# shadygm/Lichtfeld-Densification-Plugin

Measured on AMD Instinct MI355X. Metric: triangulated points/sec + pairs/sec, MipNeRF360 garden @fast, 1/2/4/8 GPU, higher is better.
Workload: dtype f32 (+f64 Sampson/DLT solve)

## Files before the change

lichtfeld-densification-plugin_amd/csrc/lfd_api.hip:

```cpp
#include <cstddef>
#include <hip/hip_runtime.h>
#include <hip/hip_ext.h>

#include <algorithm>
#include <cmath>
#include <cstdio>
#include <cstdlib>
#include <cstring>
#include <mutex>
#include <string>
#include <vector>

#include "lfd_context.hpp"

extern "C" __global__ void lfd_aggregate_kernel(LfdLaunch L, float* best_cert, uint8_t* best_slot);
extern "C" __global__ void lfd_dense_kernel(LfdLaunch L);
extern "C" __global__ void lfd_dense_exact_kernel(LfdLaunch L);
extern "C" __global__ void lfd_dense_ply_kernel(LfdLaunch L);
extern "C" __global__ void lfd_dense_ply_exact_kernel(LfdLaunch L);
extern "C" __global__ void lfd_dense_segments_kernel(LfdLaunch L);
extern "C" __global__ void lfd_dense_segments_exact_kernel(LfdLaunch L);
extern "C" __global__ void lfd_dense_ply_segments_kernel(LfdLaunch L);
extern "C" __global__ void lfd_dense_ply_segments_exact_kernel(LfdLaunch L);
extern "C" __global__ void lfd_segment_scan_kernel(const LfdTileSeg* table, int n_tiles, int tiles_per_ref, int n_refs, long long* tile_dst, long long* ref_offsets);
// ... 1370 lines not shown
    int64_t lo = key(-1.0f), hi = key(1.0f);
    while (hi - lo > 1) {
        const int64_t mid = lo + (hi - lo) / 2;
        if (ok(unkey(mid))) lo = mid; else hi = mid;
    }
    return unkey(lo);
}

int lfd_host_fundamental(const float* K1, const float* R1, const float* t1, const float* K2, const float* R2,
                         const float* t2, float* F_out) {
    if (!K1 || !R1 || !t1 || !K2 || !R2 || !t2 || !F_out) return LFD_ERR_INVALID;
    lfd_fundamental(K1, R1, t1, K2, R2, t2, F_out);
    return LFD_OK;
}

static void unpack_cam(const float* v, LfdCam& c) {
    std::memcpy(c.K, v, 9 * 4); std::memcpy(c.R, v + 9, 9 * 4); std::memcpy(c.t, v + 18, 3 * 4);
    std::memcpy(c.P, v + 21, 12 * 4); std::memcpy(c.C, v + 33, 3 * 4);
    c.w = (int32_t)v[36]; c.h = (int32_t)v[37]; c.pad[0] = c.pad[1] = 0;
}

int lfd_host_null_vector(const float* A16, double* out4) {
    if (!A16 || !out4) return -LFD_ERR_INVALID;
    return lfd_null_vector(A16, out4);
}

int lfd_host_eval_correspondence(const float* cam1, const float* cam2, float xa_norm, float ya_norm, float xb_norm,
                                 float yb_norm, int32_t w_match, int32_t h_match, const lfd_params* params, float* out8) {
    if (!cam1 || !cam2 || !params || !out8 || w_match <= 1 || h_match <= 1) return LFD_ERR_INVALID;
    LfdCam a, b;
    unpack_cam(cam1, a); unpack_cam(cam2, b);
    LfdRefConst rc; LfdPairConst pc;
    lfd_make_ref_const(a, w_match, h_match, rc);
    lfd_make_pair_const(a, b, 1, w_match, h_match, pc);
    lfd_batch bb; std::memset(&bb, 0, sizeof(bb));
    bb.w_match = w_match; bb.h_match = h_match;
    LfdKernelParams kp;
    lfd_fill_kernel_params(&bb, params, kp);
    LfdCellResult res;
    lfd_eval_correspondence(rc, pc, xa_norm, ya_norm, xb_norm, yb_norm, kp, res);
    out8[0] = res.x; out8[1] = res.y; out8[2] = res.z; out8[3] = 0.0f; out8[4] = 0.0f; out8[5] = 0.0f;
    out8[6] = res.err; out8[7] = (float)res.keep;
    return LFD_OK;
}

}
```

lichtfeld-densification-plugin_amd/csrc/lfd_geometry.hpp:

```cpp
#pragma once

#include <math.h>
#include <stdint.h>

#if defined(__HIPCC__)
#define LFD_HD __host__ __device__ __forceinline__
#else
#define LFD_HD inline
#endif
#if defined(__HIP_DEVICE_COMPILE__)
#define LFD_REREAD_CONSTANTS() asm volatile("" ::: "memory")
#define LFD_OPAQUE4(a, b, c, d) asm volatile("" : "+v"(a), "+v"(b), "+v"(c), "+v"(d) :: "memory")
#else
#define LFD_REREAD_CONSTANTS() do { } while (0)
#define LFD_OPAQUE4(a, b, c, d) do { } while (0)
#endif

struct LfdCam {
    float K[9];
    float R[9];
    float t[3];
    float P[12];
    float C[3];
    int32_t w, h;
    int32_t pad[2];
};

struct LfdRefConst {
    float P[12];
    float C[3];
    float sx, sy;
    float pad;
};

struct LfdPairConst {
    double F[9];
    float P[12];
    float C[3];
    float sx, sy;
    int32_t cam;
};

struct LfdKernelParams {
    double sampson_thresh;
    float certainty_thresh;
    float reproj_thresh;
    float dot_thresh;
    float wm1, hm1;
    int32_t use_sampson;
    int32_t use_parallax;
    int32_t no_filter;
};

struct LfdCellResult {
    float x, y, z;
    float err;
    float xa_px, ya_px;
    int32_t keep;
};

struct LfdAxis {
    float start, end, step;
    int32_t half, n;
};

LFD_HD LfdAxis lfd_make_axis(int n) {
    LfdAxis a;
    a.start = (float)(-1.0 + 1.0 / (double)n);
    a.end = (float)(1.0 - 1.0 / (double)n);
    a.step = (n > 1) ? (a.end - a.start) / (float)(n - 1) : 0.0f;
    a.half = n / 2;
    a.n = n;
    return a;
// ... 36 lines not shown
    for (int i = 0; i < 3; ++i)
        for (int j = 0; j < 3; ++j)
            R[i * 3 + j] = lfd_dot3_chain(R2[i * 3 + 0], R1[j * 3 + 0], R2[i * 3 + 1], R1[j * 3 + 1], R2[i * 3 + 2], R1[j * 3 + 2]);
    for (int i = 0; i < 3; ++i) {
        const float rt = (R[i * 3 + 0] * t1[0] + R[i * 3 + 1] * t1[1]) + R[i * 3 + 2] * t1[2];
        t[i] = t2[i] - rt;
    }
    const float S[9] = {0.0f, -t[2], t[1], t[2], 0.0f, -t[0], -t[1], t[0], 0.0f};
    for (int i = 0; i < 3; ++i)
        for (int j = 0; j < 3; ++j)
            E[i * 3 + j] = lfd_dot3_chain(S[i * 3 + 0], R[0 + j], S[i * 3 + 1], R[3 + j], S[i * 3 + 2], R[6 + j]);
    lfd_inv3_intrinsics(K1, K1i);
    lfd_inv3_intrinsics(K2, K2i);
    for (int i = 0; i < 3; ++i)
        for (int j = 0; j < 3; ++j)
            T[i * 3 + j] = lfd_dot3_chain(K2i[0 + i], E[0 + j], K2i[3 + i], E[3 + j], K2i[6 + i], E[6 + j]);
    for (int i = 0; i < 3; ++i)
        for (int j = 0; j < 3; ++j)
            F[i * 3 + j] = lfd_dot3_chain(T[i * 3 + 0], K1i[0 + j], T[i * 3 + 1], K1i[3 + j], T[i * 3 + 2], K1i[6 + j]);
}

LFD_HD void lfd_interleave_p(const float* P, float* Pi) {
    for (int c = 0; c < 4; ++c) { Pi[2 * c] = P[c]; Pi[2 * c + 1] = P[4 + c]; Pi[8 + c] = P[8 + c]; }
}

LFD_HD void lfd_make_ref_const(const LfdCam& c, int w_match, int h_match, LfdRefConst& o) {
    lfd_interleave_p(c.P, o.P);
    for (int i = 0; i < 3; ++i) o.C[i] = c.C[i];
    o.sx = (float)((double)c.w / (double)w_match);
    o.sy = (float)((double)c.h / (double)h_match);
    o.pad = 0.0f;
}

LFD_HD void lfd_make_pair_const(const LfdCam& a, const LfdCam& b, int cam_index, int w_match, int h_match,
                                LfdPairConst& o, const float* F_given = nullptr) {
    float F[9];
    if (F_given) { for (int i = 0; i < 9; ++i) F[i] = F_given[i]; }
    else lfd_fundamental(a.K, a.R, a.t, b.K, b.R, b.t, F);
    for (int i = 0; i < 9; ++i) o.F[i] = (double)F[i];
    lfd_interleave_p(b.P, o.P);
    for (int i = 0; i < 3; ++i) o.C[i] = b.C[i];
    o.sx = (float)((double)b.w / (double)w_match);
    o.sy = (float)((double)b.h / (double)h_match);
    o.cam = cam_index;
}

#ifndef LFD_PACK_ROWS
#define LFD_PACK_ROWS 0
#endif
#ifndef LFD_PARALLAX_EXACT
#define LFD_PARALLAX_EXACT 4
#endif
#ifndef LFD_NULLVEC_TOL
#define LFD_NULLVEC_TOL 1e-6
#endif
#ifndef LFD_NULLVEC_MAXIT
#define LFD_NULLVEC_MAXIT 8
#endif
#ifndef LFD_NULLVEC_PASSES
#define LFD_NULLVEC_PASSES 4
#endif

LFD_HD double lfd_pow2_inv_scale(double t) {
    int e;
    (void)frexp(t, &e);
    int es = ((t > 0.0) && (t < 1.7976931348623157e308)) ? -e : 0;
#if defined(__HIP_DEVICE_COMPILE__)
    asm volatile("" : "+v"(es));
#endif
    return ldexp(1.0, es);
}

#ifndef LFD_RCP_NEWTON_STEPS
#define LFD_RCP_NEWTON_STEPS 1
#endif
LFD_HD double lfd_sqrt_rare(double x) {
#if defined(__HIP_DEVICE_COMPILE__)
    const double r = __builtin_amdgcn_rsq(x);
    double s = x * r, h = 0.5 * r;
    double d = fma(-h, s, 0.5);
    s = fma(s, d, s); h = fma(h, d, h);
    d = fma(-s, s, x);
    s = fma(d, h, s);
    return (x > 0.0) ? s : 0.0;
#else
    return sqrt(x);
#endif
}

LFD_HD double lfd_recip_refined(double d) {
#if defined(__HIP_DEVICE_COMPILE__)
    double r = __builtin_amdgcn_rcp(d);
    r = fma(fma(-d, r, 1.0), r, r);
#if LFD_RCP_NEWTON_STEPS >= 2
    r = fma(fma(-d, r, 1.0), r, r);
#endif
    return r;
#else
    return 1.0 / d;
#endif
}

template <class RowFn>
LFD_HD int lfd_null_vector_rows(RowFn rows, double* c) {
    double m00, m01, m02, m03, m11, m12, m13, m22, m23, m33;
#define LFD_BUILD_M()                                                                                                   \
    {                                                                                                                   \
        float Af[16];                                                                                                   \
        rows(Af);                                                                                                       \
        {                                      \
            const double a0 = (double)Af[0], a1 = (double)Af[1], a2 = (double)Af[2], a3 = (double)Af[3];                \
            m00 = a0 * a0; m01 = a0 * a1; m02 = a0 * a2; m03 = a0 * a3;                                                 \
            m11 = a1 * a1; m12 = a1 * a2; m13 = a1 * a3; m22 = a2 * a2; m23 = a2 * a3; m33 = a3 * a3;                   \
        }                                                                                                               \
        _Pragma("unroll") for (int r = 1; r < 4; ++r) {                                                                 \
            const double a0 = (double)Af[4 * r + 0], a1 = (double)Af[4 * r + 1], a2 = (double)Af[4 * r + 2],            \
                         a3 = (double)Af[4 * r + 3];                                                                    \
            m00 = fma(a0, a0, m00); m01 = fma(a0, a1, m01); m02 = fma(a0, a2, m02); m03 = fma(a0, a3, m03);             \
            m11 = fma(a1, a1, m11); m12 = fma(a1, a2, m12); m13 = fma(a1, a3, m13);                                     \
            m22 = fma(a2, a2, m22); m23 = fma(a2, a3, m23); m33 = fma(a3, a3, m33);                                     \
        }                                                                                                               \
    }
    double sh = 0.0;
    double x0 = 0.0, x1 = 0.0, x2 = 0.0, x3 = 1.0;
    int it = 0;
    for (int pass = 0;; ++pass) {
        LFD_BUILD_M();
        const double q00 = m00 - sh, q11 = m11 - sh, q22 = m22 - sh, q33 = m33 - sh;
        const double r0 = lfd_recip_refined(q00);
        const double l10 = m01 * r0, l20 = m02 * r0, l30 = m03 * r0;
        const double d1 = fma(-l10, m01, q11);
        const double n12 = fma(-l10, m02, m12), n13 = fma(-l10, m03, m13);
        const double n22 = fma(-l20, m02, q22), n23 = fma(-l20, m03, m23), n33 = fma(-l30, m03, q33);
        const double r1 = lfd_recip_refined(d1);
        const double l21 = n12 * r1, l31 = n13 * r1;
        const double d2 = fma(-l21, n12, n22);
        const double p23 = fma(-l21, n13, n23), p33 = fma(-l31, n13, n33);
        const double r2 = lfd_recip_refined(d2);
        const double l32 = p23 * r2;
        const double d3 = fma(-l32, p23, p33);
        const double s0 = d3 * r0, s1 = d3 * r1, s2 = d3 * r2;
        if (pass == 0) {
            x3 = 1.0;
            x2 = -l32;
            x1 = fma(-l21, x2, -l31);
            x0 = fma(-l10, x1, fma(-l20, x2, -l30));
            it = 1;
        }
        bool settled = false;
        for (int k = 1;; ++k) {
            const double o0 = x0, o1 = x1, o2 = x2, o3 = x3;
            const double y1 = fma(-l10, x0, x1);
            const double y2 = fma(-l21, y1, fma(-l20, x0, x2));
            const double y3 = fma(-l32, y2, fma(-l31, y1, fma(-l30, x0, x3)));
            const double z0 = x0 * s0, z1 = y1 * s1, z2 = y2 * s2;
            x3 = y3;
            x2 = fma(-l32, x3, z2);
            x1 = fma(-l21, x2, fma(-l31, x3, z1));
            x0 = fma(-l10, x1, fma(-l20, x2, fma(-l30, x3, z0)));
            ++it;
            if (k >= 2) {
                const double ref = fabs(x3 * o3) * LFD_NULLVEC_TOL;
                const double e0 = fabs(fma(x0, o3, -(x3 * o0))), e1 = fabs(fma(x1, o3, -(x3 * o1))), e2 = fabs(fma(x2, o3, -(x3 * o2)));
                const bool more = (e0 > ref) || (e1 > ref) || (e2 > ref) || !(ref > 0.0);
                const bool bad = !(e0 == e0) || !(e1 == e1) || !(e2 == e2) || !(ref == ref);
                if (!more || bad) { settled = true; break; }
                if (k >= LFD_NULLVEC_MAXIT) break;
            }
        }
        if (settled || pass >= LFD_NULLVEC_PASSES - 1) break;
        LFD_BUILD_M();
        {
            const double sc = lfd_pow2_inv_scale(fabs(x0) + fabs(x1) + fabs(x2) + fabs(x3));
            x0 *= sc; x1 *= sc; x2 *= sc; x3 *= sc;
            const double t0 = fma(m03, x3, fma(m02, x2, fma(m01, x1, m00 * x0)));
            const double t1 = fma(m13, x3, fma(m12, x2, fma(m11, x1, m01 * x0)));
            const double t2 = fma(m23, x3, fma(m22, x2, fma(m12, x1, m02 * x0)));
            const double t3 = fma(m33, x3, fma(m23, x2, fma(m13, x1, m03 * x0)));
            const double num = fma(x3, t3, fma(x2, t2, fma(x1, t1, x0 * t0)));
            const double den = fma(x3, x3, fma(x2, x2, fma(x1, x1, x0 * x0)));
            const double rden = lfd_recip_refined(den);
            const double rho = num * rden;
            const double e0 = fma(-rho, x0, t0), e1 = fma(-rho, x1, t1), e2 = fma(-rho, x2, t2), e3 = fma(-rho, x3, t3);
            const double rr = fma(e3, e3, fma(e2, e2, fma(e1, e1, e0 * e0)));
            sh = rho - lfd_sqrt_rare(rr * rden);
        }
    }
    c[0] = x0; c[1] = x1; c[2] = x2; c[3] = x3;
    return it;
#undef LFD_BUILD_M
}

struct LfdCopyRows {
    const float* A;
    LFD_HD void operator()(float* Af) const { for (int i = 0; i < 16; ++i) Af[i] = A[i]; }
};
LFD_HD int lfd_null_vector(const float* Af, double* c) {
    LfdCopyRows rows{Af};
    return lfd_null_vector_rows(rows, c);
}

LFD_HD double lfd_div_by_recip(double a, double b, double r) {
    const double q = a * r;
    return fma(fma(-b, q, a), r, q);
}

LFD_HD float lfd_match_px(float n, float size_m1) {
    return ((n + 1.0f) * 0.5f) * size_m1;
}

LFD_HD float lfd_div_by_recip_f32(float a, float b, float r) {
    const float q = a * r;
    return fmaf(fmaf(-b, q, a), r, q);
}

LFD_HD float lfd_proj_row(const float* Pi, int row, float X0, float X1, float X2, float X3) {
    if (row == 2) return fmaf(X3, Pi[11], fmaf(X2, Pi[10], fmaf(X1, Pi[9], X0 * Pi[8])));
    return fmaf(X3, Pi[6 + row], fmaf(X2, Pi[4 + row], fmaf(X1, Pi[2 + row], X0 * Pi[row])));
}

// ... 15 lines not shown
LFD_HD float lfd_sqrt_rn_f32(float x) {
#if defined(__HIP_DEVICE_COMPILE__)
    const float s = __builtin_amdgcn_sqrtf(x);
    const float h = 0.5f * __builtin_amdgcn_rcpf(s);
    const float r = fmaf(-s, s, x);
    const float c = fmaf(r, h, s);
    return (x > 0.0f && x < 3.0e38f) ? c : s;
#else
    return sqrtf(x);
#endif
}
LFD_HD float lfd_rcp_rn_f32(float b) {
#if defined(__HIP_DEVICE_COMPILE__)
    const float y = __builtin_amdgcn_rcpf(b);
    return fmaf(fmaf(-b, y, 1.0f), y, y);
#else
    return 1.0f / b;
#endif
}

LFD_HD float lfd_reproj_sq(const float* P, float X0, float X1, float X2, float X3, float u, float v, float& pz) {
    const float px = lfd_proj_row(P, 0, X0, X1, X2, X3);
    const float py = lfd_proj_row(P, 1, X0, X1, X2, X3);
    pz = lfd_proj_row(P, 2, X0, X1, X2, X3);
    const float z = fmaxf(pz, 1e-12f);
    const float rz = lfd_rcp_f32(z);
    const float du = lfd_div_by_recip_f32(px, z, rz) - u;
    const float dv = lfd_div_by_recip_f32(py, z, rz) - v;
    return du * du + dv * dv;
}

LFD_HD bool lfd_finite(float x) { return fabsf(x) <= 3.402823466e+38f; }

LFD_HD void lfd_eval_correspondence(const LfdRefConst& rc, const LfdPairConst& pc, float xan, float yan,
                                    float xbn, float ybn, const LfdKernelParams& kp, LfdCellResult& o) {
    const float xa = lfd_match_px(xan, kp.wm1), ya = lfd_match_px(yan, kp.hm1);
    const float xb = lfd_match_px(xbn, kp.wm1), yb = lfd_match_px(ybn, kp.hm1);
    const float ua = xa * rc.sx, va = ya * rc.sy;
    const float ub = xb * pc.sx, vb = yb * pc.sy;
    o.xa_px = xa; o.ya_px = ya;
    o.x = o.y = o.z = 0.0f; o.err = 0.0f; o.keep = 0;

    if (kp.use_sampson) {
        const double x1 = (double)ua, y1 = (double)va, x2 = (double)ub, y2 = (double)vb;
        const double* F = pc.F;
        const double fx0 = fma(F[1], y1, fma(F[0], x1, F[2]));
        const double fx1 = fma(F[4], y1, fma(F[3], x1, F[5]));
        const double fx2 = fma(F[7], y1, fma(F[6], x1, F[8]));
        const double ft0 = fma(F[3], y2, fma(F[0], x2, F[6]));
        const double ft1 = fma(F[4], y2, fma(F[1], x2, F[7]));
        const double num = fma(x2, fx0, fma(y2, fx1, fx2));
        const double den = fma(ft1, ft1, fma(ft0, ft0, fma(fx1, fx1, fx0 * fx0))) + 1e-12;
        if (!((num * num) < kp.sampson_thresh * den)) return;
    }

    struct Rows {
        const LfdRefConst& rc; const LfdPairConst& pc; float ua, va, ub, vb;
        LFD_HD void operator()(float* A) const {
            float u1 = ua, v1 = va, u2 = ub, v2 = vb;
            LFD_OPAQUE4(u1, v1, u2, v2);
            typedef float v2f __attribute__((ext_vector_type(2)));
            const v2f uv1 = {u1, v1}, uv2 = {u2, v2};
            for (int c = 0; c < 4; ++c) {
#if LFD_PACK_ROWS & 1
                const v2f p1 = {rc.P[2 * c], rc.P[2 * c + 1]};
                const v2f m1 = uv1 * rc.P[8 + c];
                const v2f r1 = m1 - p1;
                A[0 + c] = r1.x; A[4 + c] = r1.y;
#else
                A[0 + c] = u1 * rc.P[8 + c] - rc.P[2 * c];
                A[4 + c] = v1 * rc.P[8 + c] - rc.P[2 * c + 1];
#endif
#if LFD_PACK_ROWS & 2
                const v2f p2 = {pc.P[2 * c], pc.P[2 * c + 1]};
                const v2f m2 = uv2 * pc.P[8 + c];
                const v2f r2 = m2 - p2;
                A[8 + c] = r2.x; A[12 + c] = r2.y;
#else
                A[8 + c] = u2 * pc.P[8 + c] - pc.P[2 * c];
                A[12 + c] = v2 * pc.P[8 + c] - pc.P[2 * c + 1];
#endif
            }
        }
    };
    double c[4];
#if defined(LFD_ABLATE_SOLVER)
    c[0] = ua; c[1] = va; c[2] = ub; c[3] = vb;
// ... 265 lines not shown
```

lichtfeld-densification-plugin_amd/csrc/lfd_host.hip:

```cpp
#include <algorithm>
#include <atomic>
#include <cmath>
#include <condition_variable>
#include <cstring>
#include <functional>
#include <mutex>
#include <thread>
#include <vector>

#include "lfd_context.hpp"

void lfd_fill_kernel_params(const lfd_batch* b, const lfd_params* p, LfdKernelParams& kp);

namespace {

struct HostRef {
    LfdRefConst rc;
    LfdPairConst pc[LFD_MAX_SLOTS];
};

struct HostLaunch {
    const lfd_batch* b;
    LfdKernelParams kp;
    std::vector<float> axis_x, axis_y;
// ... 92 lines not shown
        if (!b->image[r]) return lfd_fail(ctx, LFD_ERR_INVALID, "null image pointer");
        for (int j = 0; j < b->n_slots[r]; ++j) {
            const size_t s = (size_t)r * b->k + j;
            if (b->nbr_cam[s] < 0 || b->nbr_cam[s] >= n_cams) return lfd_fail(ctx, LFD_ERR_INVALID, "nbr_cam out of range");
            if (!b->cert[s] || !b->warp[s]) return lfd_fail(ctx, LFD_ERR_INVALID, "null cert/warp pointer in a valid slot");
        }
    }
    return LFD_OK;
}

void prepare_host(const lfd_batch* b, const lfd_params* p, HostLaunch& L) {
    L.b = b;
    lfd_fill_kernel_params(b, p, L.kp);
    L.HW = b->H * b->W;
    L.mask_sx = (float)b->w_match / (float)b->W;
    L.mask_sy = (float)b->h_match / (float)b->H;
    L.exact_colour = (p->flags & LFD_FLAG_EXACT_COLOUR) != 0;
    if (b->axis_x) { L.ax = b->axis_x; L.ay = b->axis_y; }
    else {
        L.axis_x.resize((size_t)b->W); L.axis_y.resize((size_t)b->H);
        const LfdAxis ax = lfd_make_axis(b->W), ay = lfd_make_axis(b->H);
        for (int j = 0; j < b->W; ++j) L.axis_x[(size_t)j] = lfd_axis_value(ax, j);
        for (int j = 0; j < b->H; ++j) L.axis_y[(size_t)j] = lfd_axis_value(ay, j);
        L.ax = L.axis_x.data(); L.ay = L.axis_y.data();
    }
}

void make_ref(const lfd_context* ctx, const HostLaunch& L, int r, HostRef& R) {
    const lfd_batch* b = L.b;
    const LfdCam& ca = ctx->host_cams[(size_t)b->ref_cam[r]];
    lfd_make_ref_const(ca, b->w_match, b->h_match, R.rc);
    for (int j = 0; j < b->n_slots[r]; ++j) {
        const size_t s = (size_t)r * b->k + j;
        lfd_make_pair_const(ca, ctx->host_cams[(size_t)b->nbr_cam[s]], b->nbr_cam[s], b->w_match, b->h_match, R.pc[j],
                            b->fundamental ? b->fundamental + s * 9 : nullptr);
    }
}

float host_cell_cert(const HostLaunch& L, int r, int j, int cell, int x, int y) {
    const lfd_batch* b = L.b;
    const size_t s = (size_t)r * b->k + j;
    float c = lfd_cert_floor(b->cert[s][cell], L.kp.certainty_thresh);
    const uint8_t* ma = b->mask_a ? b->mask_a[r] : nullptr;
    if (ma) c = c * (float)ma[(size_t)lfd_nearest_src(y, L.mask_sy, b->h_match) * b->w_match + lfd_nearest_src(x, L.mask_sx, b->w_match)];
    const uint8_t* mb = b->mask_b ? b->mask_b[s] : nullptr;
    if (mb) {
        const float* wv = b->warp[s] + (size_t)cell * b->warp_channels + (b->warp_channels - 2);
        const int ix = lfd_grid_nearest(wv[0], b->W), iy = lfd_grid_nearest(wv[1], b->H);
        float m = 0.0f;
        if (ix >= 0 && iy >= 0)
            m = (float)mb[(size_t)lfd_nearest_src(iy, L.mask_sy, b->h_match) * b->w_match + lfd_nearest_src(ix, L.mask_sx, b->w_match)];
        c = c * m;
    }
    return c;
}

void host_cell_best(const HostLaunch& L, int r, int cell, float& best, int& bj) {
    const int y = cell / L.b->W, x = cell - y * L.b->W;
    best = host_cell_cert(L, r, 0, cell, x, y);
    bj = 0;
    for (int j = 1; j < L.b->n_slots[r]; ++j) {
        const float c = host_cell_cert(L, r, j, cell, x, y);
        if ((c > best) || ((c != c) && !(best != best))) { best = c; bj = j; }
    }
}

struct HostPoint { float x, y, z, r, g, b, err; int cell; int slot; };
// ... 194 lines not shown
```

lichtfeld-densification-plugin_amd/csrc/lfd_kernels.hip:

```cpp
#include <hip/hip_runtime.h>
#include <stdint.h>

#include "lfd_device.hpp"

namespace {

constexpr int kBlock = LFD_DENSE_BLOCK;
constexpr int kCpt = LFD_DENSE_CPT;
constexpr int kTile = kBlock * kCpt;

typedef unsigned long long u64;

constexpr u64 kStEmpty = 0ull, kStAggregate = 1ull, kStPrefix = 2ull;
constexpr u64 kValueMask = (1ull << LFD_VALUE_BITS) - 1ull;
__device__ __forceinline__ u64 pack_state(u64 st, unsigned epoch, u64 v) {
    return (st << 62) | ((u64)epoch << LFD_VALUE_BITS) | (v & kValueMask);
}
__device__ __forceinline__ u64 state_status(u64 s, unsigned epoch) {
    return (((s >> LFD_VALUE_BITS) & LFD_EPOCH_MASK) == epoch) ? (s >> 62) : kStEmpty;
}

__device__ __forceinline__ void state_store(u64* p, u64 v) {
    __hip_atomic_store(p, v, __ATOMIC_RELAXED, __HIP_MEMORY_SCOPE_AGENT);
}
// ... 270 lines not shown
#pragma unroll
            for (int e = 0; e < 4; ++e) { best[e] = c[e]; bj[e] = 0; }
        } else {
#pragma unroll
            for (int e = 0; e < 4; ++e) argmax_step(c[e], j, best[e], bj[e]);
        }
    }
}

__device__ __forceinline__ void cell_coords(const LfdLaunch& L, const BlockShared& S, int cell, int bj, float& xan,
                                            float& yan, float& xbn, float& ybn) {
    const float* wp = S.slot[bj].warp;
    if (L.warp_channels == 4) {
        const float4 v = load_f32x4(wp + (size_t)cell * 4);
        xan = v.x; yan = v.y; xbn = v.z; ybn = v.w;
    } else {
        const float2 v = load_f32x2(wp + (size_t)cell * 2);
        int y, x;
        lfd_divmod(cell, L.W, L.inv_w, y, x);
        xan = lfd_global(L.axis_x)[x]; yan = lfd_global(L.axis_y)[y];
        xbn = v.x; ybn = v.y;
    }
}

}

extern "C" __global__ void lfd_pair_setup_kernel(LfdLaunch L, LfdRefConst* __restrict__ ref_out,
                                                 LfdPairConst* __restrict__ pair_out) {
    const int i = (int)(blockIdx.x * blockDim.x + threadIdx.x);
    const int n_pairs = L.n_refs * L.k;
    if (i < n_pairs) {
        const int r = i / L.k, j = i - r * L.k;
        if (j < L.refs[r].n_slots) {
            lfd_make_pair_const(L.cams[L.refs[r].cam], L.cams[L.slots[i].cam], L.slots[i].cam, L.w_match, L.h_match, pair_out[i],
                                L.fund_override ? L.fund_override + (size_t)i * 9 : nullptr);
        }
    } else if (i < n_pairs + L.n_refs) {
        const int r = i - n_pairs;
        lfd_make_ref_const(L.cams[L.refs[r].cam], L.w_match, L.h_match, ref_out[r]);
    }
}

extern "C" __global__ void __launch_bounds__(256) lfd_aggregate_kernel(LfdLaunch L, float* __restrict__ best_cert,
                                                                       uint8_t* __restrict__ best_slot) {
    __shared__ BlockShared S;
    const int r = (int)blockIdx.y;
    const int tid = (int)threadIdx.x;
    if (tid == 0) S.ref = L.refs[r];
    if (tid < L.k) S.slot[tid] = L.slots[(size_t)r * L.k + tid];
    __syncthreads();
    const int HW = L.H * L.W;
    const bool plain = !S.ref.mask_a && (HW & 3) == 0;
    bool any_mask_b = false;
    for (int j = 0; j < S.ref.n_slots; ++j) any_mask_b |= (S.slot[j].mask_b != nullptr);
    const int ns = S.ref.n_slots;
    for (int base = ((int)blockIdx.x * 256 + tid) * 4; base < HW; base += (int)gridDim.x * 256 * 4) {
        if (plain && !any_mask_b && base + 3 < HW) {
            float4 best = load_f32x4(S.slot[0].cert + base);
            const float th = L.kp.certainty_thresh;
            best.x = lfd_cert_floor(best.x, th); best.y = lfd_cert_floor(best.y, th);
            best.z = lfd_cert_floor(best.z, th); best.w = lfd_cert_floor(best.w, th);
            int b0 = 0, b1 = 0, b2 = 0, b3 = 0;
            for (int j = 1; j < ns; ++j) {
                const float4 c = load_f32x4(S.slot[j].cert + base);
                argmax_step(lfd_cert_floor(c.x, th), j, best.x, b0);
                argmax_step(lfd_cert_floor(c.y, th), j, best.y, b1);
                argmax_step(lfd_cert_floor(c.z, th), j, best.z, b2);
// ... 790 lines not shown
```

lichtfeld-densification-plugin_amd/csrc/build.py:

```python
from __future__ import annotations

import os
import shutil
import subprocess
import sys

HERE = os.path.dirname(os.path.abspath(__file__))
OUT = os.path.join(os.path.dirname(HERE), "liblfd_densify.so")
SOURCES = ["lfd_api.hip", "lfd_kernels.hip", "lfd_select.hip", "lfd_writer.hip", "lfd_host.hip", "lfd_image.hip", "lfd_voxel.hip"]
HEADERS = ["lfd_device.hpp", "lfd_geometry.hpp", "lfd_context.hpp", os.path.join("..", "..", "include", "lfd_densify.h")]
FLAGS = ["--offload-arch=gfx950", "-O3", "-std=c++17", "-ffp-contract=off", "-fPIC", "-shared",
         "-fno-fast-math", "-Wall", "-Wno-unused-function", "-pthread", "-mllvm", "-amdgpu-sched-strategy=max-ilp"]


def needs_build() -> bool:
    if not os.path.exists(OUT):
        return True
    t = os.path.getmtime(OUT)
    return any(os.path.getmtime(os.path.join(HERE, f)) > t for f in SOURCES + HEADERS + ["build.py"])


def build(force: bool = False, verbose: bool = False) -> str:
    if not force and not needs_build():
        return OUT
    hipcc = shutil.which("hipcc") or "/opt/rocm/bin/hipcc"
    cmd = [hipcc] + FLAGS + [os.path.join(HERE, s) for s in SOURCES] + ["-o", OUT]
    if verbose:
        cmd.insert(1, "-Rpass-analysis=kernel-resource-usage")
        print(" ".join(cmd))
    res = subprocess.run(cmd, capture_output=True, text=True)
    if res.returncode != 0:
        sys.stderr.write(res.stdout + res.stderr)
        raise RuntimeError("hipcc failed building liblfd_densify.so")
    if verbose:
        sys.stderr.write(res.stderr)
    return OUT


if __name__ == "__main__":
    print(build(force="--force" in sys.argv, verbose="-v" in sys.argv))
```

Before: 50.81 billion.

## Filter Sampson test in f32 with error bound, fall back to f64 when ambiguous

The Sampson epipolar check now runs first in single precision, using per-pair error-bound constants computed at pair setup. Only when the f32 margin is within a rigorous rounding bound, or the coordinates exceed the assumed range, does it recompute in f64. The aim is to avoid the slow f64 FMA chain on MI355X for most cells while keeping decisions identical. The cost is extra per-pair constants in LfdPairConst, a divergent exact path, and a tuned bound that must be correct. It also adds an ISA-mix profiling script.

```diff
diff --git a/lichtfeld-densification-plugin_amd/csrc/lfd_api.hip b/lichtfeld-densification-plugin_amd/csrc/lfd_api.hip
--- a/lichtfeld-densification-plugin_amd/csrc/lfd_api.hip
+++ b/lichtfeld-densification-plugin_amd/csrc/lfd_api.hip
@@ -1426,11 +1426,11 @@
     unpack_cam(cam1, a); unpack_cam(cam2, b);
     LfdRefConst rc; LfdPairConst pc;
     lfd_make_ref_const(a, w_match, h_match, rc);
-    lfd_make_pair_const(a, b, 1, w_match, h_match, pc);
     lfd_batch bb; std::memset(&bb, 0, sizeof(bb));
     bb.w_match = w_match; bb.h_match = h_match;
     LfdKernelParams kp;
     lfd_fill_kernel_params(&bb, params, kp);
+    lfd_make_pair_const(a, b, 1, w_match, h_match, kp.sampson_thresh, pc);
     LfdCellResult res;
     lfd_eval_correspondence(rc, pc, xa_norm, ya_norm, xb_norm, yb_norm, kp, res);
     out8[0] = res.x; out8[1] = res.y; out8[2] = res.z; out8[3] = 0.0f; out8[4] = 0.0f; out8[5] = 0.0f;
diff --git a/lichtfeld-densification-plugin_amd/csrc/lfd_geometry.hpp b/lichtfeld-densification-plugin_amd/csrc/lfd_geometry.hpp
--- a/lichtfeld-densification-plugin_amd/csrc/lfd_geometry.hpp
+++ b/lichtfeld-densification-plugin_amd/csrc/lfd_geometry.hpp
@@ -34,11 +34,13 @@
 };
 
 struct LfdPairConst {
-    double F[9];
+    float F[9];
     float P[12];
     float C[3];
     float sx, sy;
     int32_t cam;
+    float samp_r, samp_t, samp_a1, samp_a0;
+    float pad;
 };
 
 struct LfdKernelParams {
@@ -141,17 +143,39 @@
     o.pad = 0.0f;
 }
 
-LFD_HD void lfd_make_pair_const(const LfdCam& a, const LfdCam& b, int cam_index, int w_match, int h_match,
+LFD_HD void lfd_sampson_consts(const float* F, float R, double t, LfdPairConst& o) {
+    const double u = 5.9604644775390625e-08, tiny = 3.009265538105056e-36;
+    double f[9];
+    for (int i = 0; i < 9; ++i) f[i] = fabs((double)F[i]);
+    const double r = (double)R;
+    const double ax0 = r * (f[0] + f[1]) + f[2], ax1 = r * (f[3] + f[4]) + f[5], ax2 = r * (f[6] + f[7]) + f[8];
+    const double at0 = r * (f[0] + f[3]) + f[6], at1 = r * (f[1] + f[4]) + f[7];
+    const double anum = r * (ax0 + ax1) + ax2;
+    const double en = 4.03 * u * anum + tiny * (4.0 * r + 4.0);
+    const double eS = 8.1 * u * (ax0 * ax0 + ax1 * ax1 + at0 * at0 + at1 * at1) + tiny * (8.0 + 4.0 * (ax0 + ax1 + at0 + at1));
+    const double k = 1.0 + 1.0 / 1024.0;
+    o.samp_r = R;
+    o.samp_t = (float)t;
+    o.samp_a1 = (float)(2.0 * en * k);
+    o.samp_a0 = (float)((en * en + t * (eS + u * 1e-12) + tiny * (1.0 + t)) * k);
+}
+
+LFD_HD void lfd_make_pair_const(const LfdCam& a, const LfdCam& b, int cam_index, int w_match, int h_match, double sampson_thresh,
                                 LfdPairConst& o, const float* F_given = nullptr) {
     float F[9];
     if (F_given) { for (int i = 0; i < 9; ++i) F[i] = F_given[i]; }
     else lfd_fundamental(a.K, a.R, a.t, b.K, b.R, b.t, F);
-    for (int i = 0; i < 9; ++i) o.F[i] = (double)F[i];
+    for (int i = 0; i < 9; ++i) o.F[i] = F[i];
     lfd_interleave_p(b.P, o.P);
     for (int i = 0; i < 3; ++i) o.C[i] = b.C[i];
     o.sx = (float)((double)b.w / (double)w_match);
     o.sy = (float)((double)b.h / (double)h_match);
     o.cam = cam_index;
+    int m = a.w > a.h ? a.w : a.h;
+    if (b.w > m) m = b.w;
+    if (b.h > m) m = b.h;
+    lfd_sampson_consts(F, m > 0 ? 2.0f * (float)m : 0.0f, sampson_thresh, o);
+    o.pad = 0.0f;
 }
 
 #ifndef LFD_PACK_ROWS
@@ -376,6 +400,37 @@
 
 LFD_HD bool lfd_finite(float x) { return fabsf(x) <= 3.402823466e+38f; }
 
+LFD_HD bool lfd_sampson_keep(const LfdPairConst& pc, double thresh, float ua, float va, float ub, float vb, int* exact_path = nullptr) {
+    const float* Ff = pc.F;
+    const float fx0 = fmaf(Ff[1], va, fmaf(Ff[0], ua, Ff[2]));
+    const float fx1 = fmaf(Ff[4], va, fmaf(Ff[3], ua, Ff[5]));
+    const float fx2 = fmaf(Ff[7], va, fmaf(Ff[6], ua, Ff[8]));
+    const float ft0 = fmaf(Ff[3], vb, fmaf(Ff[0], ub, Ff[6]));
+    const float ft1 = fmaf(Ff[4], vb, fmaf(Ff[1], ub, Ff[7]));
+    const float num = fmaf(ub, fx0, fmaf(vb, fx1, fx2));
+    const float den = fmaf(ft1, ft1, fmaf(ft0, ft0, fmaf(fx1, fx1, fx0 * fx0))) + 1e-12f;
+    const float p = pc.samp_t * den;
+    const float d = fmaf(num, num, -p);
+    const float bound = fmaf(pc.samp_a1, fabsf(num), fmaf(4.76837158203125e-07f, p, pc.samp_a0));
+    const float mx = fmaxf(fmaxf(fabsf(ua), fabsf(va)), fmaxf(fabsf(ub), fabsf(vb)));
+    bool pass = d < 0.0f;
+    if (!((mx <= pc.samp_r) && (fabsf(d) > bound))) {
+        if (exact_path) *exact_path = 1;
+        const double x1 = (double)ua, y1 = (double)va, x2 = (double)ub, y2 = (double)vb;
+        double F[9];
+        for (int i = 0; i < 9; ++i) F[i] = (double)Ff[i];
+        const double dfx0 = fma(F[1], y1, fma(F[0], x1, F[2]));
+        const double dfx1 = fma(F[4], y1, fma(F[3], x1, F[5]));
+        const double dfx2 = fma(F[7], y1, fma(F[6], x1, F[8]));
+        const double dft0 = fma(F[3], y2, fma(F[0], x2, F[6]));
+        const double dft1 = fma(F[4], y2, fma(F[1], x2, F[7]));
+        const double dnum = fma(x2, dfx0, fma(y2, dfx1, dfx2));
+        const double dden = fma(dft1, dft1, fma(dft0, dft0, fma(dfx1, dfx1, dfx0 * dfx0))) + 1e-12;
+        pass = (dnum * dnum) < thresh * dden;
+    }
+    return pass;
+}
+
 LFD_HD void lfd_eval_correspondence(const LfdRefConst& rc, const LfdPairConst& pc, float xan, float yan,
                                     float xbn, float ybn, const LfdKernelParams& kp, LfdCellResult& o) {
     const float xa = lfd_match_px(xan, kp.wm1), ya = lfd_match_px(yan, kp.hm1);
@@ -385,18 +440,7 @@
     o.xa_px = xa; o.ya_px = ya;
     o.x = o.y = o.z = 0.0f; o.err = 0.0f; o.keep = 0;
 
-    if (kp.use_sampson) {
-        const double x1 = (double)ua, y1 = (double)va, x2 = (double)ub, y2 = (double)vb;
-        const double* F = pc.F;
-        const double fx0 = fma(F[1], y1, fma(F[0], x1, F[2]));
-        const double fx1 = fma(F[4], y1, fma(F[3], x1, F[5]));
-        const double fx2 = fma(F[7], y1, fma(F[6], x1, F[8]));
-        const double ft0 = fma(F[3], y2, fma(F[0], x2, F[6]));
-        const double ft1 = fma(F[4], y2, fma(F[1], x2, F[7]));
-        const double num = fma(x2, fx0, fma(y2, fx1, fx2));
-        const double den = fma(ft1, ft1, fma(ft0, ft0, fma(fx1, fx1, fx0 * fx0))) + 1e-12;
-        if (!((num * num) < kp.sampson_thresh * den)) return;
-    }
+    if (kp.use_sampson && !lfd_sampson_keep(pc, kp.sampson_thresh, ua, va, ub, vb)) return;
 
     struct Rows {
         const LfdRefConst& rc; const LfdPairConst& pc; float ua, va, ub, vb;
diff --git a/lichtfeld-densification-plugin_amd/csrc/lfd_host.hip b/lichtfeld-densification-plugin_amd/csrc/lfd_host.hip
--- a/lichtfeld-densification-plugin_amd/csrc/lfd_host.hip
+++ b/lichtfeld-densification-plugin_amd/csrc/lfd_host.hip
@@ -148,7 +148,7 @@
     lfd_make_ref_const(ca, b->w_match, b->h_match, R.rc);
     for (int j = 0; j < b->n_slots[r]; ++j) {
         const size_t s = (size_t)r * b->k + j;
-        lfd_make_pair_const(ca, ctx->host_cams[(size_t)b->nbr_cam[s]], b->nbr_cam[s], b->w_match, b->h_match, R.pc[j],
+        lfd_make_pair_const(ca, ctx->host_cams[(size_t)b->nbr_cam[s]], b->nbr_cam[s], b->w_match, b->h_match, L.kp.sampson_thresh, R.pc[j],
                             b->fundamental ? b->fundamental + s * 9 : nullptr);
     }
 }
diff --git a/lichtfeld-densification-plugin_amd/csrc/lfd_kernels.hip b/lichtfeld-densification-plugin_amd/csrc/lfd_kernels.hip
--- a/lichtfeld-densification-plugin_amd/csrc/lfd_kernels.hip
+++ b/lichtfeld-densification-plugin_amd/csrc/lfd_kernels.hip
@@ -326,7 +326,7 @@
     if (i < n_pairs) {
         const int r = i / L.k, j = i - r * L.k;
         if (j < L.refs[r].n_slots) {
-            lfd_make_pair_const(L.cams[L.refs[r].cam], L.cams[L.slots[i].cam], L.slots[i].cam, L.w_match, L.h_match, pair_out[i],
+            lfd_make_pair_const(L.cams[L.refs[r].cam], L.cams[L.slots[i].cam], L.slots[i].cam, L.w_match, L.h_match, L.kp.sampson_thresh, pair_out[i],
                                 L.fund_override ? L.fund_override + (size_t)i * 9 : nullptr);
         }
     } else if (i < n_pairs + L.n_refs) {
diff --git a/profiles/isa_mix.py b/profiles/isa_mix.py
--- /dev/null
+++ b/profiles/isa_mix.py
@@ -0,0 +1,91 @@
+#!/usr/bin/env python3
+import argparse
+import collections
+import os
+import re
+import sys
+
+CLASSES = ("f64", "f32", "cvt", "int", "trans", "mov", "cndmask", "cmp", "other")
+TRANS = ("rcp", "rsq", "sqrt", "exp", "log", "sin", "cos", "frexp", "ldexp")
+
+
+def vclass(op):
+    if not op.startswith("v_"):
+        return None
+    if op.startswith(("v_cmp", "v_cmpx")):
+        return "cmp"
+    if op.startswith("v_cndmask"):
+        return "cndmask"
+    if op.startswith(("v_mov", "v_readfirstlane", "v_readlane", "v_writelane", "v_accvgpr", "v_swap")):
+        return "mov"
+    if op.startswith("v_cvt"):
+        return "cvt"
+    body = op[2:]
+    if any(body.startswith(t) for t in TRANS):
+        return "trans"
+    if "_f64" in op:
+        return "f64"
+    if "_f32" in op or "_f16" in op:
+        return "f32"
+    if re.search(r"_(u|i|b)(16|24|32|64)", op) or op.startswith(("v_lshl", "v_lshr", "v_ashr", "v_and", "v_or", "v_xor", "v_not", "v_bfe", "v_bfi", "v_alignbit", "v_perm", "v_mbcnt", "v_bcnt")):
+        return "int"
+    return "other"
+
+
+def kernel_lines(path, kernel):
+    lines = open(path).read().splitlines()
+    start = next(i for i, l in enumerate(lines) if l.startswith(kernel + ":"))
+    end = next(i for i in range(start, len(lines)) if lines[i].strip().startswith(".Lfunc_end") and lines[i].strip().endswith(":"))
+    meta = {}
+    for l in lines[end:end + 400]:
+        m = re.match(r"\s*;\s*(NumVgprs|ScratchSize|NumSgprs|Occupancy|LDSByteSize|SGPRBlocks|VGPRBlocks)\s*:\s*(\S+)", l)
+        if m and m.group(1) not in meta:
+            meta[m.group(1)] = m.group(2)
+    return lines[start:end], meta
+
+
+def mix(lines, between=None):
+    c = collections.Counter()
+    on = between is None
+    spills = 0
+    for l in lines:
+        s = l.strip()
+        if between and s.startswith(between[0]):
+            on = True
+        if between and s.startswith(between[1]):
+            on = False
+        if not on or not s or s.startswith((";", ".")) or s.endswith(":"):
+            continue
+        op = s.split()[0]
+        if op.startswith("v_writelane") or "spill" in s.lower():
+            spills += 1
+        k = vclass(op)
+        if k:
+            c[k] += 1
+            c["total"] += 1
+    return c, spills
+
+
+def main():
+    ap = argparse.ArgumentParser()
+    ap.add_argument("asm")
+    ap.add_argument("--kernel", default="lfd_dense_kernel")
+    ap.add_argument("--diff")
+    ap.add_argument("--between", nargs=2)
+    a = ap.parse_args()
+    files = [a.asm] + ([a.diff] if a.diff else [])
+    rows = []
+    for f in files:
+        lines, meta = kernel_lines(f, a.kernel)
+        c, spills = mix(lines, a.between)
+        rows.append(c)
+        print(f"{f}: {a.kernel}  VGPRs {meta.get('NumVgprs')}  scratch {meta.get('ScratchSize')}  LDS {meta.get('LDSByteSize')}  "
+              f"occupancy {meta.get('Occupancy')}  spill/writelane lines {spills}")
+    print("class    " + "".join(f"{os.path.basename(f)[:12]:>14s}" for f in files) + ("          diff" if a.diff else ""))
+    for k in CLASSES + ("total",):
+        v = [r.get(k, 0) for r in rows]
+        print(f"{k:8s} " + "".join(f"{x:14d}" for x in v) + (f"{v[1] - v[0]:+14d}" if a.diff else ""))
+
+
+if __name__ == "__main__":
+    sys.exit(main())
```

Result: no change. 51.08 billion, median of 6 (+0.5%).

## Unroll first inverse-iteration pass and compile kernels with SLP vectorisation disabled

Applied to the files above, without the earlier changes.

The null-vector solver's first pass is written out explicitly: it factorises once without a shift, runs the first iterations in ping-pong registers, and only then falls into the generic loop. Later shifted passes become a separate loop, so the pass-0 branch and the shift arithmetic are removed from the hot path. The build now compiles each source separately and in parallel, adding -fno-slp-vectorize for lfd_kernels.hip, which avoids packed-f32 instructions that a new microbenchmark is meant to evaluate. This adds code size, and changing vectorisation could alter register pressure or scheduling.

```diff
diff --git a/lichtfeld-densification-plugin_amd/csrc/build.py b/lichtfeld-densification-plugin_amd/csrc/build.py
--- a/lichtfeld-densification-plugin_amd/csrc/build.py
+++ b/lichtfeld-densification-plugin_amd/csrc/build.py
@@ -4,13 +4,22 @@
 import shutil
 import subprocess
 import sys
+import tempfile
+from concurrent.futures import ThreadPoolExecutor
 
 HERE = os.path.dirname(os.path.abspath(__file__))
 OUT = os.path.join(os.path.dirname(HERE), "liblfd_densify.so")
 SOURCES = ["lfd_api.hip", "lfd_kernels.hip", "lfd_select.hip", "lfd_writer.hip", "lfd_host.hip", "lfd_image.hip", "lfd_voxel.hip"]
 HEADERS = ["lfd_device.hpp", "lfd_geometry.hpp", "lfd_context.hpp", os.path.join("..", "..", "include", "lfd_densify.h")]
-FLAGS = ["--offload-arch=gfx950", "-O3", "-std=c++17", "-ffp-contract=off", "-fPIC", "-shared",
+FLAGS = ["--offload-arch=gfx950", "-O3", "-std=c++17", "-ffp-contract=off", "-fPIC",
          "-fno-fast-math", "-Wall", "-Wno-unused-function", "-pthread", "-mllvm", "-amdgpu-sched-strategy=max-ilp"]
+FILE_FLAGS = {"lfd_kernels.hip": ["-fno-slp-vectorize"]}
+LINK_FLAGS = ["--offload-arch=gfx950", "-fPIC", "-shared", "-pthread"]
+
+
+def compile_command(source: str, out: str, extra=()) -> list:
+    hipcc = shutil.which("hipcc") or "/opt/rocm/bin/hipcc"
+    return [hipcc] + FLAGS + FILE_FLAGS.get(source, []) + list(extra) + ["-c", os.path.join(HERE, source), "-o", out]
 
 
 def needs_build() -> bool:
@@ -24,16 +33,25 @@
     if not force and not needs_build():
         return OUT
     hipcc = shutil.which("hipcc") or "/opt/rocm/bin/hipcc"
-    cmd = [hipcc] + FLAGS + [os.path.join(HERE, s) for s in SOURCES] + ["-o", OUT]
-    if verbose:
-        cmd.insert(1, "-Rpass-analysis=kernel-resource-usage")
-        print(" ".join(cmd))
-    res = subprocess.run(cmd, capture_output=True, text=True)
-    if res.returncode != 0:
-        sys.stderr.write(res.stdout + res.stderr)
-        raise RuntimeError("hipcc failed building liblfd_densify.so")
-    if verbose:
-        sys.stderr.write(res.stderr)
+    extra = ["-Rpass-analysis=kernel-resource-usage"] if verbose else []
+    with tempfile.TemporaryDirectory(prefix="lfd_build_") as tmp:
+        objs = [os.path.join(tmp, os.path.splitext(f)[0] + ".o") for f in SOURCES]
+        cmds = [compile_command(f, o, extra) for f, o in zip(SOURCES, objs)]
+        with ThreadPoolExecutor(max_workers=min(len(cmds), int(os.environ.get("MAX_JOBS", "8")))) as pool:
+            results = list(pool.map(lambda c: subprocess.run(c, capture_output=True, text=True), cmds))
+        link = [hipcc] + LINK_FLAGS + objs + ["-o", OUT]
+        for cmd, res in zip(cmds, results):
+            if verbose:
+                print(" ".join(cmd))
+            if res.returncode != 0:
+                sys.stderr.write(res.stdout + res.stderr)
+                raise RuntimeError("hipcc failed building liblfd_densify.so (" + os.path.basename(cmd[-3]) + ")")
+            if verbose:
+                sys.stderr.write(res.stderr)
+        res = subprocess.run(link, capture_output=True, text=True)
+        if res.returncode != 0:
+            sys.stderr.write(res.stdout + res.stderr)
+            raise RuntimeError("hipcc failed linking liblfd_densify.so")
     return OUT
 
 
diff --git a/lichtfeld-densification-plugin_amd/csrc/lfd_geometry.hpp b/lichtfeld-densification-plugin_amd/csrc/lfd_geometry.hpp
--- a/lichtfeld-densification-plugin_amd/csrc/lfd_geometry.hpp
+++ b/lichtfeld-densification-plugin_amd/csrc/lfd_geometry.hpp
@@ -208,6 +208,14 @@
 #else
     return 1.0 / d;
 #endif
+}
+
+LFD_HD bool lfd_nullvec_settled(double n0, double n1, double n2, double n3, double o0, double o1, double o2, double o3) {
+    const double ref = fabs(n3 * o3) * LFD_NULLVEC_TOL;
+    const double e0 = fabs(fma(n0, o3, -(n3 * o0))), e1 = fabs(fma(n1, o3, -(n3 * o1))), e2 = fabs(fma(n2, o3, -(n3 * o2)));
+    const bool more = (e0 > ref) || (e1 > ref) || (e2 > ref) || !(ref > 0.0);
+    const bool bad = !(e0 == e0) || !(e1 == e1) || !(e2 == e2) || !(ref == ref);
+    return !more || bad;
 }
 
 template <class RowFn>
@@ -230,54 +238,69 @@
             m22 = fma(a2, a2, m22); m23 = fma(a2, a3, m23); m33 = fma(a3, a3, m33);                                     \
         }                                                                                                               \
     }
-    double sh = 0.0;
-    double x0 = 0.0, x1 = 0.0, x2 = 0.0, x3 = 1.0;
-    int it = 0;
-    for (int pass = 0;; ++pass) {
+#define LFD_FACTORISE(q00, q11, q22, q33)                                                                               \
+    const double r0 = lfd_recip_refined(q00);                                                                           \
+    const double l10 = m01 * r0, l20 = m02 * r0, l30 = m03 * r0;                                                        \
+    const double d1 = fma(-l10, m01, q11);                                                                              \
+    const double n12 = fma(-l10, m02, m12), n13 = fma(-l10, m03, m13);                                                  \
+    const double n22 = fma(-l20, m02, q22), n23 = fma(-l20, m03, m23), n33 = fma(-l30, m03, q33);                       \
+    const double r1 = lfd_recip_refined(d1);                                                                            \
+    const double l21 = n12 * r1, l31 = n13 * r1;                                                                        \
+    const double d2 = fma(-l21, n12, n22);                                                                              \
+    const double p23 = fma(-l21, n13, n23), p33 = fma(-l31, n13, n33);                                                  \
+    const double r2 = lfd_recip_refined(d2);                                                                            \
+    const double l32 = p23 * r2;                                                                                        \
+    const double d3 = fma(-l32, p23, p33);                                                                              \
+    const double s0 = d3 * r0, s1 = d3 * r1, s2 = d3 * r2
+#define LFD_SOLVE(a0, a1, a2, a3, b0, b1, b2, b3)                                                                       \
+    {                                                                                                                   \
+        const double y1 = fma(-l10, a0, a1);                                                                            \
+        const double y2 = fma(-l21, y1, fma(-l20, a0, a2));                                                             \
+        const double y3 = fma(-l32, y2, fma(-l31, y1, fma(-l30, a0, a3)));                                              \
+        const double z0 = a0 * s0, z1 = y1 * s1, z2 = y2 * s2;                                                          \
+        b3 = y3;                                                                                                        \
+        b2 = fma(-l32, b3, z2);                                                                                         \
+        b1 = fma(-l21, b2, fma(-l31, b3, z1));                                                                          \
+        b0 = fma(-l10, b1, fma(-l20, b2, fma(-l30, b3, z0)));                                                           \
+    }
+#if LFD_NULLVEC_MAXIT < 4
+#error "pass 0 of lfd_null_vector_rows is written out for LFD_NULLVEC_MAXIT >= 4"
+#endif
+    double x0, x1, x2, x3;
+    int it;
+    bool settled;
+    {
         LFD_BUILD_M();
-        const double q00 = m00 - sh, q11 = m11 - sh, q22 = m22 - sh, q33 = m33 - sh;
-        const double r0 = lfd_recip_refined(q00);
-        const double l10 = m01 * r0, l20 = m02 * r0, l30 = m03 * r0;
-        const double d1 = fma(-l10, m01, q11);
-        const double n12 = fma(-l10, m02, m12), n13 = fma(-l10, m03, m13);
-        const double n22 = fma(-l20, m02, q22), n23 = fma(-l20, m03, m23), n33 = fma(-l30, m03, q33);
-        const double r1 = lfd_recip_refined(d1);
-        const double l21 = n12 * r1, l31 = n13 * r1;
-        const double d2 = fma(-l21, n12, n22);
-        const double p23 = fma(-l21, n13, n23), p33 = fma(-l31, n13, n33);
-        const double r2 = lfd_recip_refined(d2);
-        const double l32 = p23 * r2;
-        const double d3 = fma(-l32, p23, p33);
-        const double s0 = d3 * r0, s1 = d3 * r1, s2 = d3 * r2;
-        if (pass == 0) {
-            x3 = 1.0;
-            x2 = -l32;
-            x1 = fma(-l21, x2, -l31);
-            x0 = fma(-l10, x1, fma(-l20, x2, -l30));
-            it = 1;
-        }
-        bool settled = false;
-        for (int k = 1;; ++k) {
-            const double o0 = x0, o1 = x1, o2 = x2, o3 = x3;
-            const double y1 = fma(-l10, x0, x1);
-            const double y2 = fma(-l21, y1, fma(-l20, x0, x2));
-            const double y3 = fma(-l32, y2, fma(-l31, y1, fma(-l30, x0, x3)));
-            const double z0 = x0 * s0, z1 = y1 * s1, z2 = y2 * s2;
-            x3 = y3;
-            x2 = fma(-l32, x3, z2);
-            x1 = fma(-l21, x2, fma(-l31, x3, z1));
-            x0 = fma(-l10, x1, fma(-l20, x2, fma(-l30, x3, z0)));
-            ++it;
-            if (k >= 2) {
-                const double ref = fabs(x3 * o3) * LFD_NULLVEC_TOL;
-                const double e0 = fabs(fma(x0, o3, -(x3 * o0))), e1 = fabs(fma(x1, o3, -(x3 * o1))), e2 = fabs(fma(x2, o3, -(x3 * o2)));
-                const bool more = (e0 > ref) || (e1 > ref) || (e2 > ref) || !(ref > 0.0);
-                const bool bad = !(e0 == e0) || !(e1 == e1) || !(e2 == e2) || !(ref == ref);
-                if (!more || bad) { settled = true; break; }
-                if (k >= LFD_NULLVEC_MAXIT) break;
+        LFD_FACTORISE(m00, m11, m22, m33);
+        x3 = 1.0;
+        x2 = -l32;
+        x1 = fma(-l21, x2, -l31);
+        x0 = fma(-l10, x1, fma(-l20, x2, -l30));
+        double w0, w1, w2, w3;
+        LFD_SOLVE(x0, x1, x2, x3, w0, w1, w2, w3);
+        LFD_SOLVE(w0, w1, w2, w3, x0, x1, x2, x3);
+        it = 3;
+        settled = lfd_nullvec_settled(x0, x1, x2, x3, w0, w1, w2, w3);
+        if (!settled) {
+            LFD_SOLVE(x0, x1, x2, x3, w0, w1, w2, w3);
+            it = 4;
+            settled = lfd_nullvec_settled(w0, w1, w2, w3, x0, x1, x2, x3);
+            if (settled) { x0 = w0; x1 = w1; x2 = w2; x3 = w3; }
+            else {
+                LFD_SOLVE(w0, w1, w2, w3, x0, x1, x2, x3);
+                it = 5;
+                settled = lfd_nullvec_settled(x0, x1, x2, x3, w0, w1, w2, w3);
+                for (int k = 5; !settled && k <= LFD_NULLVEC_MAXIT; ++k) {
+                    const double o0 = x0, o1 = x1, o2 = x2, o3 = x3;
+                    LFD_SOLVE(x0, x1, x2, x3, x0, x1, x2, x3);
+                    ++it;
+                    settled = lfd_nullvec_settled(x0, x1, x2, x3, o0, o1, o2, o3);
+                }
             }
         }
-        if (settled || pass >= LFD_NULLVEC_PASSES - 1) break;
+    }
+    for (int pass = 1; !settled && pass < LFD_NULLVEC_PASSES; ++pass) {
+        double sh;
         LFD_BUILD_M();
         {
             const double sc = lfd_pow2_inv_scale(fabs(x0) + fabs(x1) + fabs(x2) + fabs(x3));
@@ -294,7 +317,17 @@
             const double rr = fma(e3, e3, fma(e2, e2, fma(e1, e1, e0 * e0)));
             sh = rho - lfd_sqrt_rare(rr * rden);
         }
-    }
+        LFD_BUILD_M();
+        LFD_FACTORISE(m00 - sh, m11 - sh, m22 - sh, m33 - sh);
+        for (int k = 1; k <= LFD_NULLVEC_MAXIT; ++k) {
+            const double o0 = x0, o1 = x1, o2 = x2, o3 = x3;
+            LFD_SOLVE(x0, x1, x2, x3, x0, x1, x2, x3);
+            ++it;
+            if (k >= 2 && lfd_nullvec_settled(x0, x1, x2, x3, o0, o1, o2, o3)) { settled = true; break; }
+        }
+    }
+#undef LFD_FACTORISE
+#undef LFD_SOLVE
     c[0] = x0; c[1] = x1; c[2] = x2; c[3] = x3;
     return it;
 #undef LFD_BUILD_M
diff --git a/profiles/microbench/fma_f32_packing.hip b/profiles/microbench/fma_f32_packing.hip
--- /dev/null
+++ b/profiles/microbench/fma_f32_packing.hip
@@ -0,0 +1,81 @@
+#include <hip/hip_runtime.h>
+#include <cstdio>
+#include <cstdlib>
+
+#define CHK(x) do { hipError_t e = (x); if (e != hipSuccess) { fprintf(stderr, "%s: %s\n", #x, hipGetErrorString(e)); exit(1); } } while (0)
+
+constexpr int kIters = 4096;
+constexpr int kChains = 8;
+typedef float v2f __attribute__((ext_vector_type(2)));
+
+template <int OP>
+__global__ void __launch_bounds__(256) chain_kernel(double* out, float seed, int iters) {
+    float f[kChains];
+    v2f p[kChains];
+    double d[kChains], e[kChains];
+    for (int i = 0; i < kChains; ++i) {
+        f[i] = seed + i + threadIdx.x;
+        p[i] = v2f{f[i], f[i] + 0.5f};
+        d[i] = (double)f[i];
+        e[i] = d[i] + 1.0;
+    }
+    const float fm = seed * 0.999f, fc = seed * 0.5f;
+    const v2f pm = {fm, fm}, pc = {fc, fc};
+    const double dm = (double)fm, dc = (double)fc;
+    for (int it = 0; it < iters; ++it) {
+#pragma unroll
+        for (int i = 0; i < kChains; ++i) {
+            if (OP == 0) asm volatile("v_fma_f32 %0, %0, %1, %2" : "+v"(f[i]) : "v"(fm), "v"(fc));
+            if (OP == 1) asm volatile("v_pk_fma_f32 %0, %0, %1, %2" : "+v"(p[i]) : "v"(pm), "v"(pc));
+            if (OP == 2) asm volatile("v_mul_f32 %0, %0, %1" : "+v"(f[i]) : "v"(fm));
+            if (OP == 3) asm volatile("v_pk_mul_f32 %0, %0, %1" : "+v"(p[i]) : "v"(pm));
+            if (OP == 4) asm volatile("v_fma_f64 %0, %0, %1, %2" : "+v"(d[i]) : "v"(dm), "v"(dc));
+            if (OP == 5) asm volatile("v_mov_b64 %0, %1" : "=v"(e[i]) : "v"(d[i]));
+            if (OP == 6) asm volatile("v_max_f64 %0, %0, %1" : "+v"(d[i]) : "v"(dm));
+            if (OP == 7) asm volatile("v_cmp_gt_f64 vcc, %0, %1" :: "v"(d[i]), "v"(dm) : "vcc");
+        }
+    }
+    double s = 0.0;
+    for (int i = 0; i < kChains; ++i) s += (double)f[i] + (double)p[i].x + (double)p[i].y + d[i] + e[i];
+    if (s == 1.2345e-300) out[0] = s;
+}
+
+template <int OP>
+double run(const char* name, int waves_per_simd) {
+    hipDeviceProp_t p; CHK(hipGetDeviceProperties(&p, 0));
+    const int blocks = p.multiProcessorCount * waves_per_simd;
+    double* d; CHK(hipMalloc(&d, 8));
+    hipEvent_t e0, e1; CHK(hipEventCreate(&e0)); CHK(hipEventCreate(&e1));
+    chain_kernel<OP><<<blocks, 256>>>(d, 1.000001f, 16);
+    CHK(hipDeviceSynchronize());
+    float best = 1e30f;
+    for (int rep = 0; rep < 5; ++rep) {
+        CHK(hipEventRecord(e0));
+        chain_kernel<OP><<<blocks, 256>>>(d, 1.000001f, kIters);
+        CHK(hipEventRecord(e1)); CHK(hipEventSynchronize(e1));
+        float ms; CHK(hipEventElapsedTime(&ms, e0, e1));
+        if (ms < best) best = ms;
+    }
+    const double insts = (double)kIters * kChains * waves_per_simd;
+    const double clk = (double)p.clockRate * 1e3;
+    const double cyc = best * 1e-3 * clk / insts;
+    printf("%-14s waves/SIMD %d  %.3f ms  %.2f cycles per wave-instruction (at %.0f MHz nominal)\n", name, waves_per_simd, best, cyc, clk / 1e6);
+    CHK(hipEventDestroy(e0)); CHK(hipEventDestroy(e1)); CHK(hipFree(d));
+    return cyc;
+}
+
+int main() {
+    for (int w : {1, 2, 4, 8}) {
+        const double s = run<0>("v_fma_f32", w);
+        const double k = run<1>("v_pk_fma_f32", w);
+        run<2>("v_mul_f32", w);
+        run<3>("v_pk_mul_f32", w);
+        run<4>("v_fma_f64", w);
+        run<5>("v_mov_b64", w);
+        run<6>("v_max_f64", w);
+        run<7>("v_cmp_gt_f64", w);
+        printf("  waves/SIMD %d: one v_pk_fma_f32 costs %.2f scalar v_fma_f32 (two scalar ones do the same work: packed is %s)\n", w, k / s,
+               k < 2.0 * s ? "cheaper per f32 operation" : "no cheaper per f32 operation");
+    }
+    return 0;
+}
```

After: 51.71 billion before, 53.30 billion after (median of 6 runs). 1.03x the previous value.
